# RishWijewardhena/vision-textile-inspection

Measured on AMD Instinct MI355X. Metric: frames/sec whole-node, YOLOv8n-seg 640x640 bs=64; mask IoU vs CPU ref, higher is better.
Workload: dtype f16x2

## Files before the change

vision-textile-inspection_amd/csrc/conv.hip:

```cpp
#include <algorithm>
#include <cstdlib>
#include <type_traits>

#include "conv_dev.h"

namespace vti {

__host__ __device__ inline int patch_dim(int t, int ks, int s, int mode) { return mode == 1 ? t : (t - 1) * s + ks; }

size_t stem_lds_bytes(int TH, int TW);

bool conv_wreg_ok(int ks, int stride, int mode, int WN, int NREP, int threads) {
    return mode == 0 && ks == 1 && stride == 1 && threads == 256 && WN == 4 && NREP <= 4;
}

size_t conv_lds_bytes(int ks, int stride, int mode, int TH, int TW, int WN, int NREP, int wreg) {
    if (mode == 1) return stem_lds_bytes(TH, TW);
    const int npix = patch_dim(TH, ks, stride, mode) * patch_dim(TW, ks, stride, mode);
    const size_t plane = (size_t)((npix + 15) & ~15) * 16;
    const int taps = mode == 1 ? 1 : ks * ks;
    size_t raw = 0;
    if (mode == 1) raw = (((size_t)(2 * TH + 1) * (2 * TW + 1) * 3) + 15) & ~(size_t)15;
    return 4 * plane + (wreg ? 0 : (size_t)WN * NREP * taps * 1024) + raw;
}

template <typename T, int KS, int S, int NREP, int WN, int NREP2 = 0, int NT = 256, bool WREG = false>
__global__ __launch_bounds__(NT, NT == 512 ? 1 : 2) void conv_kernel(const ConvParams p) {
    using vec = typename Tr<T>::vec;
    constexpr int VEC = Tr<T>::VEC, KC = Tr<T>::KC;
    constexpr int TAPS = KS * KS, PAD = KS / 2;
    constexpr int NTB = WN * NREP;
    constexpr int PP = NT / 4;
    constexpr int AR = NT == 512 ? 6 : (S == 2 ? 12 : 8);
    constexpr int BR = (NTB * TAPS * 64 + NT - 1) / NT;
    static_assert(!WREG || (KS == 1 && WN == NT / 64 && NREP2 == 0 && BR == NREP && NREP < 5), "WREG: one consumer wave per fragment");
    constexpr unsigned OOB = 0xFFFFFFFFu;
    extern __shared__ __attribute__((aligned(16))) char smem[];

    const int tid = threadIdx.x, lane = tid & 63, wave = tid >> 6;
    const int wn = wave % WN, wm = wave / WN;
    int t = blockIdx.x;
    const int tx = t % p.tiles_x; t /= p.tiles_x;
    const int ty = t % p.tiles_y;
// ... 127 lines not shown
        if (c < 2) VTI_STAMP(5 + 5 * c);
        if (c + 1 < p.nchunks) __syncthreads();
    };

    issue(0, ra[0], rb[0]);
    if constexpr (PD == 2) {
        if (p.nchunks > 1) issue(1, ra[1], rb[1]);
        for (int c = 0; c < p.nchunks; c += 2) {
            chunk(c, std::integral_constant<int, 0>{});
            if (c + 1 < p.nchunks) chunk(c + 1, std::integral_constant<int, 1>{});
        }
    } else {
        for (int c = 0; c < p.nchunks; ++c) chunk(c, std::integral_constant<int, 0>{});
    }

    VTI_STAMP(11);
    if constexpr (NREP2 == 0) {
        conv_epilogue<T, NREP>(p, acc, pvalid, opy, opx, b, nt0, wn, lane);
    } else {
        static_assert(WN == 1, "fused stage needs the whole Cout in one wave");
        conv_stage2<T, NREP, NREP2>(p, acc, pvalid, opy, opx, b, lane);
    }
    VTI_STAMP(12);
}

size_t convfold_lds_bytes(int TH, int TW) {
    const int npix = (TH + 2) * (TW + 2);
    return 4 * (size_t)((npix + 15) & ~15) * 16 + (size_t)16 * 4 * 1024;
}
bool convfold_supported(int c_in, int c_mid, int c_out, int ntiles2) {
    return c_in == c_mid && c_mid % 16 == 0 && c_out == 64 && c_in % 16 == 0 && c_in <= 64 && combo_has(FoldN2{}, ntiles2);
}

template <typename T, int NREP2, int NT = 256>
__global__ __launch_bounds__(NT, NT == 512 ? 1 : 2) void convfold_kernel(const ConvParams p) {
    using vec = typename Tr<T>::vec;
    constexpr int VEC = Tr<T>::VEC, KC = Tr<T>::KC;
    constexpr int NREP = 4, TAPS = 4, NTB = 16, AR = 8;
    constexpr int BR = NTB * TAPS * 64 / NT;
    constexpr int PPP = NT / 4;
    constexpr unsigned OOB = 0xFFFFFFFFu;
    extern __shared__ __attribute__((aligned(16))) char smem[];

    const int tid = threadIdx.x, lane = tid & 63, wave = (tid >> 6) & 3, mgrp = tid >> 8;
    const int py = wave >> 1, px = wave & 1;
    int t = blockIdx.x;
    const int tx = t % p.tiles_x; t /= p.tiles_x;
    const int ty = t % p.tiles_y;
    const int b = t / p.tiles_y;
    const int oy0 = ty * p.TH, ox0 = tx * p.TW;
    const int PH = p.TH + 2, PW = p.TW + 2;
    const int npix = PH * PW;
    const int plane_bytes = ((npix + 15) & ~15) * 16;
    char* smA = smem;
    char* smB = smem + 4 * plane_bytes;
    const int tile_px = p.TH * p.TW;

    int abase[MREP], opy[MREP], opx[MREP];
    bool pvalid[MREP];
#pragma unroll
    for (int m = 0; m < MREP; ++m) {
        const int pp = (mgrp * MREP + m) * 16 + (lane & 15);
        const bool v = pp < tile_px;
        const int pc = v ? pp : 0;
        const int ly = (int)__umulhi((unsigned)pc, p.tw_magic), lx = pc - ly * p.TW;
        pvalid[m] = v && oy0 + ly < p.Hout && ox0 + lx < p.Wout;
        opy[m] = 2 * (oy0 + ly) + py; opx[m] = 2 * (ox0 + lx) + px;
        abase[m] = (lane >> 4) * plane_bytes + ((ly + py) * PW + lx + px) * 16;
    }
    f32x4 acc[MREP][NREP];
#pragma unroll
    for (int m = 0; m < MREP; ++m)
#pragma unroll
        for (int n = 0; n < NREP; ++n) acc[m][n] = (f32x4){0.f, 0.f, 0.f, 0.f};

    const size_t frame_elems = (size_t)p.Hin * p.Win * p.in_ld;
    const __amdgpu_buffer_rsrc_t rsA = __builtin_amdgcn_make_buffer_rsrc(
        (void*)((const T*)p.in + (size_t)b * frame_elems), 0, (int)(frame_elems * sizeof(T)), 0x00020000);
    const __amdgpu_buffer_rsrc_t rsB = __builtin_amdgcn_make_buffer_rsrc((void*)p.wpk, 0, (int)p.wpk_bytes, 0x00020000);
    const int iy0 = oy0 - 1, ix0 = ox0 - 1;
    const int q = (tid >> 3) & 3;
    const int pix0 = (tid >> 5) * 8 + (tid & 7);
    const int ldsA0 = q * plane_bytes + pix0 * 16;
    const int cvalid = (p.Cin - q * VEC + KC - 1) / KC;
    unsigned aoff[AR];
#pragma unroll
    for (int u = 0; u < AR; ++u) {
        const int pix = pix0 + PPP * u;
        const int ry = (int)__umulhi((unsigned)pix, p.pw_magic), rx = pix - ry * PW;
        const int y = iy0 + ry, x = ix0 + rx;
        const bool ok = pix < npix && (unsigned)y < (unsigned)p.Hin && (unsigned)x < (unsigned)p.Win;
        aoff[u] = ok ? (unsigned)(((y * p.Win + x) * p.in_ld + p.in_coff + q * VEC) * (int)sizeof(T)) : OOB;
    }
    vec ra[AR];
    auto issue = [&](int c) {
        const bool qok = c < cvalid;
#pragma unroll
        for (int u = 0; u < AR; ++u)
            if (pix0 + PPP * u < ((npix + 7) & ~7))
                ra[u] = buf_load16<vec>(rsA, qok ? aoff[u] : OOB, (unsigned)(c * KC * (int)sizeof(T)));
    };
    auto commit = [&](int c) {
        const unsigned sB = (unsigned)((size_t)c * (NTB * TAPS * 1024));
#pragma unroll
        for (int h = 0; h < 2; ++h) {
            vec rb[BR / 2];
#pragma unroll
            for (int u = 0; u < BR / 2; ++u) rb[u] = buf_load16<vec>(rsB, (unsigned)(tid + (h * (BR / 2) + u) * NT) * 16u, sB);
            if (h == 0) {
#pragma unroll
                for (int u = 0; u < AR; ++u)
                    if (pix0 + PPP * u < npix) *(vec*)(smA + ldsA0 + u * (PPP * 16)) = ra[u];
            }
#pragma unroll
            for (int u = 0; u < BR / 2; ++u) *(vec*)(smB + (tid + (h * (BR / 2) + u) * NT) * 16) = rb[u];
        }
    };

    issue(0);
    for (int c = 0; c < p.nchunks; ++c) {
        commit(c);
        __syncthreads();
        if (c + 1 < p.nchunks) issue(c + 1);
        {
            constexpr int NSTEP = TAPS * MREP;
            vec xq[3];
            vec wq[2][NREP];
            auto ldx = [&](int s_) -> vec {
                const int tp = s_ / MREP, mm = s_ % MREP;
                return *(const vec*)(smA + abase[mm] + ((tp >> 1) * PW + (tp & 1)) * 16);
            };
            auto ldw = [&](int tp, vec (&w)[NREP]) {
#pragma unroll
                for (int n = 0; n < NREP; ++n) w[n] = *(const vec*)(smB + ((wave * NREP + n) * TAPS + tp) * 1024 + lane * 16);
            };
            if constexpr (Tr<T>::H2) {
                auto ldw1 = [&](int tp, int n) -> vec { return *(const vec*)(smB + ((wave * NREP + n) * TAPS + tp) * 1024 + lane * 16); };
                h2_taps<NREP, MREP, TAPS, 3>(acc, ldx, ldw1);
            } else {
            ldw(0, wq[0]);
            xq[0] = ldx(0);
            xq[1] = ldx(1);
#pragma unroll
            for (int s_ = 0; s_ < NSTEP; ++s_) {
                const int tp = s_ / MREP, mm = s_ % MREP;
                if (s_ + 2 < NSTEP) xq[(s_ + 2) % 3] = ldx(s_ + 2);
                if (mm == 0 && tp + 1 < TAPS) ldw(tp + 1, wq[(tp + 1) % 2]);
                __builtin_amdgcn_sched_barrier(0);
#pragma unroll
                for (int n = 0; n < NREP; ++n) acc[mm][n] = mma(wq[tp % 2][n], xq[s_ % 3], acc[mm][n]);
                __builtin_amdgcn_sched_barrier(0);
            }
            }
        }
        if (c + 1 < p.nchunks) __syncthreads();
    }
    conv_stage2<T, NREP, NREP2, true>(p, acc, pvalid, opy, opx, b, lane);
}

hipError_t launch_convfold(int dtype, const ConvParams& p, size_t lds_bytes, hipStream_t st) {
    dim3 grid((unsigned)(p.B * p.tiles_y * p.tiles_x));
    if (grid.x == 0) return hipSuccess;
    const int nthr = p.nt == 512 ? 512 : 256;
    if (p.TH * p.TW > (nthr / 256) * MREP * 16 || ((p.TH + 2) * (p.TW + 2) + 7) / 8 * 32 > nthr * 8 || p.Cout != 256 || !p.out2 || !p.fold)
        return hipErrorInvalidValue;
    return with_conv_type(dtype, [&](auto t) -> hipError_t {
        using T = typename decltype(t)::type;
        if (p.nt == 512) {
            if constexpr (sizeof(T) == 4)
                return combo_dispatch(FoldN2{}, [&](auto c) {
                    return launch_lds<convfold_kernel<T, decltype(c)::v[0], 512>>(grid, dim3(512), lds_bytes, st, p);
                }, p.ntiles2);
            return hipErrorInvalidValue;
        }
        return combo_dispatch(FoldN2{}, [&](auto c) {
            return launch_lds<convfold_kernel<T, decltype(c)::v[0]>>(grid, dim3(256), lds_bytes, st, p);
        }, p.ntiles2);
    });
}

template <typename T, int NREP>
__global__ __launch_bounds__(256) void stem_kernel(const ConvParams p) {
    using vec = typename Tr<T>::vec;
    constexpr int VEC = Tr<T>::VEC, KC = Tr<T>::KC;
    constexpr int NCH = 32 / KC;
    extern __shared__ __attribute__((aligned(16))) char smem[];
    T* lut = (T*)smem;
    unsigned* raw32 = (unsigned*)(smem + 1024);
    const unsigned char* raw = (const unsigned char*)raw32;

    const int tid = threadIdx.x, lane = tid & 63, wave = tid >> 6;
    int t = blockIdx.x;
    const int tx = t % p.tiles_x; t /= p.tiles_x;
    const int ty = t % p.tiles_y;
    const int b = t / p.tiles_y;
    const int oy0 = ty * p.TH, ox0 = tx * p.TW;
    const int RH = 2 * p.TH + 1, RWB = (2 * p.TW + 1) * 3;
    const int RWD = (RWB + 6) >> 2;
    const int pitch = RWD * 4;
    const int x0b = (ox0 * 2 - 1) * 3, a0 = x0b & ~3, shift = x0b - a0;
    const int y0 = oy0 * 2 - 1;
    const uint8_t* inb = (const uint8_t*)p.in + (size_t)b * p.Hin * p.Win * 3;
    const int rowbytes = p.Win * 3;
    if ((rowbytes & 3) == 0 && RH * RWD <= 8 * 256) {
// ... 50 lines not shown
    f32x4 acc[MREP][NREP];
#pragma unroll
    for (int m = 0; m < MREP; ++m)
#pragma unroll
        for (int n = 0; n < NREP; ++n) acc[m][n] = (f32x4){0.f, 0.f, 0.f, 0.f};
#pragma unroll
    for (int c = 0; c < NCH; ++c) {
        int off[VEC];
#pragma unroll
        for (int j = 0; j < VEC; ++j) {
            const int k = c * KC + (lane >> 4) * VEC + j;
            const int tap = k / 3, chn = k - tap * 3;
            const int kh = tap / 3, kw = tap - kh * 3;
            off[j] = k < 27 ? kh * pitch + kw * 3 + (p.swap_rb ? 2 - chn : chn) : -1;
        }
        vec w[NREP];
#pragma unroll
        for (int n = 0; n < NREP; ++n) {
            const int nt = nt0 + n < p.ntiles_n ? nt0 + n : 0;
            w[n] = ((const vec*)p.wpk)[((size_t)c * p.ntiles_n + nt) * 64 + lane];
        }
#pragma unroll
        for (int m = 0; m < MREP; ++m) {
            vec x;
#pragma unroll
            for (int j = 0; j < VEC; ++j) vset<T>(x, j, off[j] >= 0 ? lut[raw[rbase[m] + off[j]]] : to_T<T>(0.f));
#pragma unroll
            for (int n = 0; n < NREP; ++n) acc[m][n] = mma(w[n], x, acc[m][n]);
        }
    }
    conv_epilogue<T, NREP>(p, acc, pvalid, opy, opx, b, nt0, 0, lane);
}

constexpr int SL_TH = 8, SL_TW = 40;
constexpr int SL_SH = 2 * SL_TH + 1, SL_SW = 2 * SL_TW + 1, SL_NSP = SL_SH * SL_SW;
constexpr int SL_RH = 4 * SL_TH + 3, SL_RWB = (4 * SL_TW + 3) * 3, SL_RWD = (SL_RWB + 6) >> 2;
constexpr int sl_pitch(int es) { return es == 2 ? 520 : 512; }
constexpr int SL_NJ = (SL_SW + 3) / 4, SL_NWIN = SL_SH * SL_NJ;
static_assert(24 * (SL_NJ - 1) + 32 <= 512 && SL_RWD * 4 <= 512, "stem windows must stay inside a patch row");

size_t stem_l1_lds_bytes(int dtype) {
    const size_t es = dtype == VTI_F16 ? 2 : 4, pes = dtype == VTI_F32 ? 4 : 2;
    return (((size_t)SL_RH * sl_pitch((int)pes) * pes + 15) & ~(size_t)15) + (size_t)SL_NSP * 16 * es;
}

template <typename T>
__global__ __launch_bounds__(256, sizeof(T) == 2 ? 2 : 1) void stem_l1_kernel(const ConvParams p) {
    using vec = typename Tr<T>::vec;
    constexpr int ES = (int)sizeof(T);
    constexpr bool XH = Tr<T>::H2;
    using PT = typename std::conditional<XH, half_t, T>::type;
    using pvec = typename Tr<PT>::vec;
    constexpr int VEC = Tr<PT>::VEC, KC = Tr<PT>::KC, PES = (int)sizeof(PT);
    constexpr int NCH = 32 / KC;
    constexpr int NWP = XH ? 2 : 1;
    constexpr int NS1 = sizeof(T) == 2 ? 5 : 9;
    constexpr bool FAST = !Tr<T>::F32;
    constexpr int SL_PITCH = sl_pitch(PES);
    constexpr int CP_BYTES = (SL_RH * SL_PITCH * PES + 15) & ~15;
    extern __shared__ __attribute__((aligned(16))) char smem[];
    PT* cp = (PT*)smem;
    char* sout = smem + CP_BYTES;

    const int tid = threadIdx.x, lane = tid & 63, wave = tid >> 6, g = lane >> 4;
    const int ntiles = p.B * p.tiles_y * p.tiles_x;
    if ((int)blockIdx.x >= ntiles) return;
    const int Hs = (p.Hin - 1) / 2 + 1, Ws = (p.Win - 1) / 2 + 1;
    const int rowbytes = p.Win * 3;
    auto tile_geom = [&](int tt, int& b_, int& oy0_, int& ox0_) {
        const int tx = tt % p.tiles_x, r = tt / p.tiles_x;
        b_ = r / p.tiles_y; oy0_ = (r % p.tiles_y) * SL_TH; ox0_ = tx * SL_TW;
    };
    VTI_STAMP(0);
    constexpr int RC = (SL_RWD + 63) / 64, NR = (SL_RH + 3) / 4;
    unsigned vv[NR][RC];
    const bool aligned = (rowbytes & 3) == 0;
    auto issue_raw = [&](int tt) {
        int b_, oy0_, ox0_;
        tile_geom(tt, b_, oy0_, ox0_);
        const int iy0_ = 2 * (2 * oy0_ - 1) - 1, a0_ = ((2 * (2 * ox0_ - 1) - 1) * 3) & ~3;
        const uint8_t* inb_ = (const uint8_t*)p.in + (size_t)b_ * p.Hin * p.Win * 3;
#pragma unroll
        for (int it = 0; it < NR; ++it) {
            const int ry = wave + 4 * it;
            const int y = iy0_ + ry;
            const bool row_ok = ry < SL_RH && (unsigned)y < (unsigned)p.Hin;
#pragma unroll
            for (int ch = 0; ch < RC; ++ch) {
                const int rd = lane + 64 * ch;
                const int gx = a0_ + 4 * rd;
                const bool ok = row_ok && rd < SL_RWD && gx >= 0 && gx < rowbytes;
                vv[it][ch] = *(const unsigned*)(inb_ + (ok ? (size_t)y * rowbytes + gx : (size_t)0));
            }
        }
    };
    if (aligned) issue_raw((int)blockIdx.x);
    for (int t = (int)blockIdx.x; t < ntiles; t += (int)gridDim.x) {
    int b, oy0, ox0;
    tile_geom(t, b, oy0, ox0);
    const int sy0 = 2 * oy0 - 1, sx0 = 2 * ox0 - 1;
    const int iy0 = 2 * sy0 - 1;
    const int x0b = (2 * sx0 - 1) * 3, a0 = x0b & ~3;
    const uint8_t* inb = (const uint8_t*)p.in + (size_t)b * p.Hin * p.Win * 3;
    const void* w0p = p.w0;
    const void* w1p = p.wpk;
    asm volatile("" : "+s"(w0p), "+s"(w1p));
    pvec wA[4][3][NCH * NWP];
    {
        const pvec* w0 = (const pvec*)w0p + (size_t)(p.swap_rb ? 1 : 0) * (4 * 3 * NCH * NWP * 64);
#pragma unroll
        for (int pp = 0; pp < 4; ++pp)
#pragma unroll
            for (int kh = 0; kh < 3; ++kh)
#pragma unroll
                for (int c = 0; c < NCH * NWP; ++c) wA[pp][kh][c] = w0[(size_t)((pp * 3 + kh) * NCH * NWP + c) * 64 + lane];
    }
    vec w1all[NS1][2];
#pragma unroll
    for (int s1 = 0; s1 < NS1; ++s1)
#pragma unroll
        for (int n = 0; n < 2; ++n) w1all[s1][n] = ((const vec*)w1p)[((size_t)s1 * 2 + n) * 64 + lane];
    const f32x4 bias0_4 = *(const f32x4*)(p.bias0 + g * 4);
    Stage2Regs<T, 2, 2> s2r;
    if (p.out2) stage2_preload<T, 2, 2>(p, lane, false, s2r);
    {
        if (aligned) {
#pragma unroll
            for (int it = 0; it < NR; ++it) {
                const int ry = wave + 4 * it;
// ... 23 lines not shown
                        for (int k = 0; k < 4; ++k)
                            if (gx + k >= 0 && gx + k < rowbytes) v |= (unsigned)inb[(size_t)y * rowbytes + gx + k] << (8 * k);
                    }
                    vv[it][ch] = v;
                }
            }
        }
#pragma unroll
        for (int it = 0; it < NR; ++it) {
            const int ry = wave + 4 * it;
#pragma unroll
            for (int ch = 0; ch < RC; ++ch) {
                const int rd = lane + 64 * ch;
                if (ry >= SL_RH || rd >= SL_RWD) continue;
                const unsigned v = vv[it][ch];
                PT* o = cp + (size_t)ry * SL_PITCH + 4 * rd;
                if constexpr (XH) {
                    half4 hv;
#pragma unroll
                    for (int k = 0; k < 4; ++k) hv[k] = (half_t)(float)((v >> (8 * k)) & 0xffu);
                    *(half4*)o = hv;
                } else if constexpr (sizeof(T) == 2) {
                    half4 hv;
#pragma unroll
                    for (int k = 0; k < 4; ++k) hv[k] = (half_t)((float)((v >> (8 * k)) & 0xffu) * (1.0f / 255.0f));
                    *(half4*)o = hv;
                } else {
#pragma unroll
                    for (int k = 0; k < 4; ++k) o[k] = to_T<T>((float)((v >> (8 * k)) & 0xffu) / 255.0f);
                }
            }
        }
    }
    for (int i = tid; i < SL_RH * ((SL_PITCH - 4 * SL_RWD) / 4); i += 256) {
        const int ry = i / ((SL_PITCH - 4 * SL_RWD) / 4), c4 = i - ry * ((SL_PITCH - 4 * SL_RWD) / 4);
        PT* o = cp + (size_t)ry * SL_PITCH + 4 * SL_RWD + 4 * c4;
        o[0] = to_T<PT>(0.f); o[1] = to_T<PT>(0.f); o[2] = to_T<PT>(0.f); o[3] = to_T<PT>(0.f);
    }
    __syncthreads();
    VTI_STAMP(1);
    if (aligned && t + (int)gridDim.x < ntiles) issue_raw(t + (int)gridDim.x);
    {
        const f32x4 bias4 = bias0_4;
        constexpr int NBLK = (SL_NWIN + 15) / 16;
        for (int blk = wave; blk < NBLK; blk += 4) {
            const int wi = blk * 16 + (lane & 15);
            const bool wvalid = wi < SL_NWIN;
            const int wc = wvalid ? wi : SL_NWIN - 1;
            const int J = wc / SL_SH, sy = wc - J * SL_SH;
            const PT* base = cp + (size_t)(2 * sy) * SL_PITCH + 24 * J + g * VEC;
            pvec x[3][NCH];
#pragma unroll
            for (int kh = 0; kh < 3; ++kh)
#pragma unroll
                for (int c = 0; c < NCH; ++c) x[kh][c] = *(const pvec*)(base + kh * SL_PITCH + c * KC);
            f32x4 acc[4];
#pragma unroll
            for (int pp = 0; pp < 4; ++pp) {
                acc[pp] = (f32x4){0.f, 0.f, 0.f, 0.f};
#pragma unroll
                for (int kh = 0; kh < 3; ++kh)
#pragma unroll
                    for (int c = 0; c < NCH; ++c)
#pragma unroll
                        for (int wp = 0; wp < NWP; ++wp) acc[pp] = mma(wA[pp][kh][c * NWP + wp], x[kh][c], acc[pp]);
            }
            const bool row_in = (unsigned)(sy0 + sy) < (unsigned)Hs;
#pragma unroll
            for (int pp = 0; pp < 4; ++pp) {
                const int sx = 4 * J + pp;
                f32x4 v = silu4<FAST>(acc_bias<T>(acc[pp], bias4, p.alpha0));
                if (!(row_in && (unsigned)(sx0 + sx) < (unsigned)Ws)) v = (f32x4){0.f, 0.f, 0.f, 0.f};
                if (wvalid && sx < SL_SW) {
                    T* o = (T*)(sout + ((size_t)(sy * SL_SW + sx) * 16 + g * 4) * ES);
                    if constexpr (sizeof(T) == 2) {
                        half4 hv;
#pragma unroll
                        for (int j = 0; j < 4; ++j) hv[j] = (half_t)v[j];
                        *(half4*)o = hv;
                    } else {
                        *(u32x4*)o = pack4<T>(v);
                    }
                }
            }
        }
    }
    __syncthreads();
    VTI_STAMP(2);
    int opy[MREP], opx[MREP], sbase[MREP];
    bool pvalid[MREP];
#pragma unroll
    for (int m = 0; m < MREP; ++m) {
        const int pp = (wave * MREP + m) * 16 + (lane & 15);
        const int py = pp / SL_TW, px = pp - py * SL_TW;
        opy[m] = oy0 + py; opx[m] = ox0 + px;
        pvalid[m] = opy[m] < p.Hout && opx[m] < p.Wout;
        sbase[m] = ((2 * py) * SL_SW + 2 * px) * 16 * ES;
    }
    f32x4 acc[MREP][2];
#pragma unroll
    for (int m = 0; m < MREP; ++m) { acc[m][0] = (f32x4){0.f, 0.f, 0.f, 0.f}; acc[m][1] = (f32x4){0.f, 0.f, 0.f, 0.f}; }
#pragma unroll
    for (int s = 0; s < NS1; ++s) {
        const int tap = sizeof(T) == 2 ? 2 * s + (g >> 1) : s;
        const int tc = tap < 9 ? tap : 8;
        const int toff = ((tc / 3) * SL_SW + (tc % 3)) * 16 * ES + (sizeof(T) == 2 ? (g & 1) * 8 : g * 4) * ES;
        vec w1[2];
#pragma unroll
        for (int n = 0; n < 2; ++n) w1[n] = w1all[s][n];
#pragma unroll
        for (int m = 0; m < MREP; ++m) {
            const vec x = *(const vec*)(sout + sbase[m] + toff);
#pragma unroll
            for (int n = 0; n < 2; ++n) acc[m][n] = mma(w1[n], x, acc[m][n]);
        }
    }
    VTI_STAMP(3);
    if (p.out2) conv_stage2<T, 2, 2, false, true>(p, acc, pvalid, opy, opx, b, lane, &s2r);
    else conv_epilogue<T, 2>(p, acc, pvalid, opy, opx, b, 0, 0, lane);
    VTI_STAMP(12);
    }
}

void stem_l1_tile(int* th, int* tw) { *th = SL_TH; *tw = SL_TW; }

int stem_l1_grid(int dtype, int ntiles, bool persistent) {
    const int wgpc = (int)std::min<size_t>(2, (160 * 1024) / stem_l1_lds_bytes(dtype));
    if (!persistent) return ntiles;
    return std::min(ntiles, 256 * std::max(1, wgpc));
}

hipError_t launch_stem_l1(int dtype, const ConvParams& p, hipStream_t st, bool persistent) {
    dim3 grid((unsigned)stem_l1_grid(dtype, p.B * p.tiles_y * p.tiles_x, persistent));
    if (grid.x == 0) return hipSuccess;
    const size_t lds = stem_l1_lds_bytes(dtype);
    return with_conv_type(dtype, [&](auto t) { return launch_lds<stem_l1_kernel<typename decltype(t)::type>>(grid, dim3(256), lds, st, p); });
}

size_t stem_lds_bytes(int TH, int TW) { return 1024 + (size_t)(2 * TH + 1) * ((((2 * TW + 1) * 3 + 6) >> 2) * 4); }

using ConvTile3 = Combos<Ints<1, 1>, Ints<2, 1>, Ints<3, 1>, Ints<4, 1>, Ints<5, 1>, Ints<1, 2>, Ints<2, 2>, Ints<1, 4>>;
using ConvTile1 = decltype(concat(ConvTile3{}, Combos<Ints<3, 2>, Ints<4, 2>, Ints<5, 2>, Ints<2, 4>, Ints<3, 4>, Ints<4, 4>, Ints<5, 4>>{}));
using ConvTile1W = Combos<Ints<1, 4>, Ints<2, 4>, Ints<3, 4>, Ints<4, 4>>;
using StemNrep = Combos<Ints<1>, Ints<2>, Ints<3>, Ints<4>, Ints<5>>;

// ... 66 lines not shown
```

vision-textile-inspection_amd/csrc/conv_dev.h:

```cpp
#pragma once
#include "vti_internal.h"

namespace vti {

typedef _Float16 half_t;
typedef _Float16 half8 __attribute__((ext_vector_type(8)));
typedef _Float16 half4 __attribute__((ext_vector_type(4)));
typedef float f32x4 __attribute__((ext_vector_type(4)));

typedef unsigned u32x4 __attribute__((ext_vector_type(4)));

struct h2_t { unsigned u; };
struct h2x4 { u32x4 u; };
constexpr float H2_SX = 16.0f;

template <typename T> struct Tr;
template <> struct Tr<half_t> { typedef half8 vec; static constexpr int VEC = 8, KC = 32; static constexpr bool H16 = true, F32 = false, H2 = false; };
template <> struct Tr<float> { typedef f32x4 vec; static constexpr int VEC = 4, KC = 16; static constexpr bool H16 = false, F32 = true, H2 = false; };
template <> struct Tr<h2_t> { typedef h2x4 vec; static constexpr int VEC = 4, KC = 16; static constexpr bool H16 = false, F32 = false, H2 = true; };

typedef _Float16 half2v __attribute__((ext_vector_type(2)));
__device__ __forceinline__ unsigned h2_enc(float v) {
    half2v p;
    p[0] = (half_t)__builtin_fmaf(v, H2_SX, 0.0f);
// ... 316 lines not shown
                } else {
                    v += unpack4<T>(*(const u32x4*)rp);
                }
            }
            const size_t o = opix * p.out_ld + p.out_coff + co;
            if (p.scalar_store) {
#pragma unroll
                for (int j = 0; j < 4; ++j) {
                    if (cout0 + j < p.Cout) {
                        if (p.out_f32) ((float*)p.out)[o + j] = v[j];
                        else if constexpr (Tr<T>::H2) ((unsigned*)p.out)[o + j] = h2_enc(v[j]);
                        else ((T*)p.out)[o + j] = (T)v[j];
                    }
                }
            } else if (p.out_f32 || Tr<T>::F32) {
                *(f32x4*)((float*)p.out + o) = v;
            } else if constexpr (Tr<T>::H2) {
                *(u32x4*)((unsigned*)p.out + o) = pack4<T>(v);
            } else {
                half4 hv;
#pragma unroll
                for (int j = 0; j < 4; ++j) hv[j] = (half_t)v[j];
                *(half4*)((half_t*)p.out + o) = hv;
            }
        }
    }
}

template <typename V> __device__ __forceinline__ V buf_load16(__amdgpu_buffer_rsrc_t r, unsigned voff, unsigned soff) {
    const u32x4 v = __builtin_amdgcn_raw_buffer_load_b128(r, voff, soff, 0);
    return __builtin_bit_cast(V, v);
}

template <typename T, int NREP, int NREP2> struct Stage2Regs {
    using vec = typename Tr<T>::vec;
    static constexpr int KT = sizeof(T) == 2 ? (NREP + 1) / 2 : NREP;
    vec w2[KT][NREP2];
    f32x4 bias1[NREP];
    f32x4 bias2[NREP2];
};

template <typename T, int NREP, int NREP2>
__device__ __forceinline__ void stage2_preload(const ConvParams& p, int lane, bool fold, Stage2Regs<T, NREP, NREP2>& r) {
    using vec = typename Tr<T>::vec;
    const __amdgpu_buffer_rsrc_t rsW2 = __builtin_amdgcn_make_buffer_rsrc(
        (void*)p.w2, 0, (int)(Stage2Regs<T, NREP, NREP2>::KT * p.ntiles2 * 1024), 0x00020000);
#pragma unroll
    for (int t2 = 0; t2 < Stage2Regs<T, NREP, NREP2>::KT; ++t2)
#pragma unroll
        for (int n = 0; n < NREP2; ++n) r.w2[t2][n] = buf_load16<vec>(rsW2, (unsigned)(((t2 * p.ntiles2 + n) * 64 + lane) * 16), 0u);
    const float* b1 = p.bias + (fold ? 4 * (16 * NREP) : 0) + (lane >> 4) * 4 * NREP;
#pragma unroll
    for (int n = 0; n < NREP; ++n) r.bias1[n] = *(const f32x4*)(b1 + 4 * n);
    const int crun2 = p.nat2 ? (lane >> 4) * 4 : (lane >> 4) * 4 * NREP2, cstep2 = p.nat2 ? 16 : 4;
#pragma unroll
    for (int n = 0; n < NREP2; ++n) r.bias2[n] = *(const f32x4*)(p.bias2 + crun2 + cstep2 * n);
}

template <typename T, int NREP, int NREP2, bool FOLD = false, bool PRE = false>
__device__ __forceinline__ void conv_stage2(const ConvParams& p, f32x4 (&acc)[MREP][NREP], const bool (&pvalid)[MREP],
                                            const int (&opy)[MREP], const int (&opx)[MREP], int b, int lane,
                                            const Stage2Regs<T, NREP, NREP2>* pre = nullptr, bool interior = false) {
    const int OW = FOLD ? 2 * p.Wout : p.Wout;
    using vec = typename Tr<T>::vec;
    constexpr bool FAST = !Tr<T>::F32;
    constexpr int KT = sizeof(T) == 2 ? (NREP + 1) / 2 : NREP;
// ... 215 lines not shown
```

vision-textile-inspection_amd/csrc/conv_pk.hip:

```cpp
#include <algorithm>
#include <cstdlib>
#include <type_traits>

#include "conv_dev.h"

namespace vti {

constexpr int PK_PWP = 24;
constexpr int PK_TW = 20;
constexpr int PK_ROWS = 4;
constexpr int PK_MAXD = 9;
constexpr int PK_MAXD2 = 13;

using ConvPkS1 = Combos<Ints<1, 1>, Ints<2, 1>, Ints<3, 1>, Ints<4, 1>, Ints<5, 1>, Ints<1, 2>, Ints<2, 2>, Ints<3, 2>, Ints<4, 2>, Ints<1, 4>,
                        Ints<2, 4>>;
using ConvPkS2 = Combos<Ints<1, 4>, Ints<2, 2>, Ints<4, 1>, Ints<2, 1>, Ints<1, 2>>;
using Conv1Pk = decltype(concat(ConvPkS1{}, Combos<Ints<4, 4>>{}));
bool conv_pk_instantiated(int nrep, int wn) { return combo_has(ConvPkS1{}, nrep, wn); }
bool conv_pk2_instantiated(int nrep, int wn) { return combo_has(ConvPkS2{}, nrep, wn); }
bool conv1_pk_instantiated(int nrep, int wn) { return combo_has(Conv1Pk{}, nrep, wn); }
using Conv1PkWH2 = Combos<Ints<2, 2, 4>, Ints<2, 2, 6>, Ints<2, 2, 8>, Ints<2, 2, 12>, Ints<2, 2, 16>,
                          Ints<2, 4, 4>, Ints<2, 4, 6>, Ints<2, 4, 8>, Ints<2, 4, 12>, Ints<2, 4, 16>>;
using Conv1PkWF16 = Combos<Ints<2, 2, 2>, Ints<2, 2, 3>, Ints<2, 2, 4>, Ints<2, 2, 6>, Ints<2, 2, 8>,
                           Ints<2, 4, 2>, Ints<2, 4, 3>, Ints<2, 4, 4>, Ints<2, 4, 6>, Ints<2, 4, 8>, Ints<4, 1, 2>>;
// ... 5 lines not shown

static size_t pk_stage_bytes(int TH, int S) { return S == 2 ? (size_t)(2 * TH + 1) * 2 * PK_PWP * 64 : (size_t)(TH + 2) * PK_PWP * 64; }
static size_t pk3_lds_bytes(int S, int TH, int WN, int NREP, int nchunks, int depth, int wstat) {
    const int nwbuf = wstat ? nchunks : nchunks > 2 ? depth : (nchunks > 1 ? 2 : 1);
    return depth * pk_stage_bytes(TH, S) + (size_t)nwbuf * WN * NREP * 9 * 1024 + (size_t)WN * NREP * 16 * 4;
}
static bool pk3_fits(int S, int TH, int WN, int NREP, int nchunks, int wstat) {
    if (TH % PK_ROWS || (S == 2 && !conv_pk2_instantiated(NREP, WN))) return false;
    const int ncomp = (TH / PK_ROWS) * WN;
    if (ncomp < 1 || ncomp > 4) return false;
    const int ndma = (int)(pk_stage_bytes(TH, S) / 1024);
    if ((ndma + ncomp - 1) / ncomp > (S == 2 ? PK_MAXD2 : PK_MAXD)) return false;
    return pk3_lds_bytes(S, TH, WN, NREP, nchunks, 2, wstat) <= 160 * 1024;
}
template <typename F>
static int pk_ring_depth(int maxd, int per_step, F lds_at) {
    int d = 2;
    while (d < maxd && lds_at(d + 1) <= 160 * 1024 && per_step * (d - 1) <= 63) ++d;
    return d;
}
static int pk3_depth(int S, int TH, int WN, int NREP, int nchunks, int wstat, int maxd) {
    if (!pk3_fits(S, TH, WN, NREP, nchunks, wstat)) return 0;
    const int ncomp = (TH / PK_ROWS) * WN;
    const int per_step = ((int)(pk_stage_bytes(TH, S) / 1024) + ncomp - 1) / ncomp + (nchunks > 2 && !wstat ? (WN * NREP * 9 + ncomp - 1) / ncomp : 0);
    return pk_ring_depth(maxd, per_step, [&](int d) { return pk3_lds_bytes(S, TH, WN, NREP, nchunks, d, wstat); });
}
size_t conv_pk_lds_bytes(int TH, int WN, int NREP, int nchunks, int depth, int wstat) { return pk3_lds_bytes(1, TH, WN, NREP, nchunks, depth, wstat); }
size_t conv_pk2_lds_bytes(int TH, int WN, int NREP, int nchunks, int depth, int wstat) { return pk3_lds_bytes(2, TH, WN, NREP, nchunks, depth, wstat); }
bool conv_pk_fits(int TH, int WN, int NREP, int nchunks, int wstat) { return pk3_fits(1, TH, WN, NREP, nchunks, wstat); }
bool conv_pk2_fits(int TH, int WN, int NREP, int nchunks, int wstat) { return pk3_fits(2, TH, WN, NREP, nchunks, wstat); }
int conv_pk_depth(int TH, int WN, int NREP, int nchunks, int wstat, int maxd) { return pk3_depth(1, TH, WN, NREP, nchunks, wstat, maxd); }
int conv_pk2_depth(int TH, int WN, int NREP, int nchunks, int wstat, int maxd) { return pk3_depth(2, TH, WN, NREP, nchunks, wstat, maxd); }

__device__ __forceinline__ void dma16(__amdgpu_buffer_rsrc_t r, unsigned voff, unsigned soff, unsigned lds_addr) {
    unsigned keep;
    asm volatile("s_mov_b32 %0, m0\n\ts_mov_b32 m0, %1\n\ts_nop 0\n\tbuffer_load_dwordx4 %2, %3, %4 offen lds\n\ts_mov_b32 m0, %0"
                 : "=&s"(keep) : "s"(lds_addr), "v"(voff), "s"(r), "s"(soff) : "memory");
}

template <int N> __device__ __forceinline__ void wait_vm() { asm volatile("s_waitcnt vmcnt(%0)" :: "i"(N) : "memory"); }
template <int N> struct WaitVm { static __device__ __forceinline__ void go(int n) { if (n >= N) wait_vm<N>(); else WaitVm<N - 1>::go(n); } };
template <> struct WaitVm<0> { static __device__ __forceinline__ void go(int) { wait_vm<0>(); } };

__device__ __forceinline__ void pk_stagger_wait(int units) {
    if (units > 0 && (int)(blockIdx.x >> 3) * 2 >= (int)(gridDim.x >> 3))
        for (int i = 0; i < units; ++i) __builtin_amdgcn_s_sleep(16);
}

template <typename T, int NREP, int WN, int NREP2 = 0, bool FOLD = false, int S = 1>
__global__ __launch_bounds__(512) void conv3_pk(const ConvParams p) {
    using vec = typename Tr<T>::vec;
    constexpr int VEC = Tr<T>::VEC, KC = Tr<T>::KC, ES = (int)sizeof(T);
    constexpr int TAPS = FOLD ? 4 : 9, NTB = WN * NREP;
    constexpr int PWP = S == 2 ? 2 * PK_PWP : PK_PWP;
    constexpr int MAXD = S == 2 ? PK_MAXD2 : PK_MAXD;
    static_assert(S == 1 || (S == 2 && !FOLD && NREP2 == 0), "stride 2: plain epilogue only");
    constexpr int WCHUNK = NTB * TAPS * 1024;
    constexpr unsigned OOB = 0x80000000u;
    constexpr bool FAST = !Tr<T>::F32;
    extern __shared__ __attribute__((aligned(16))) char smem[];

    const int tid = threadIdx.x, lane = tid & 63;
    const int wave = __builtin_amdgcn_readfirstlane(tid >> 6);
    static_assert(!FOLD || (WN == 4 && NREP2 > 0), "fold: one compute wave per output phase, fused 1x1 epilogue");
    const int ncomp = (p.TH / PK_ROWS) * WN;
    const int nld = (int)(blockDim.x >> 6) - ncomp;
    const int PH = S == 2 ? 2 * p.TH + 1 : p.TH + 2;
    const int stage_bytes = PH * PWP * 64;
    const int ndma = PH * PWP / 16;
    const int D = p.pk_depth;
    const bool stream_w = p.nchunks > 2 && !p.pk_wstat;
    const int wbuf_off = D * stage_bytes;
    const int bias_off = wbuf_off + (stream_w ? D : p.nchunks) * WCHUNK;
// ... 1195 lines not shown
```

vision-textile-inspection_amd/csrc/vti_api.cpp:

```cpp
#include <algorithm>
#include <cmath>
#include <cstdio>
#include <cstdlib>
#include <cstring>
#include <new>

#include "vti_internal.h"
#include "rawframes_dev.h"

using namespace vti;

struct vti_ctx {
    Options opt;
    Plan plan;
    std::string err;
    int device = -1;
    void* d_wpk = nullptr;
    float* d_bias = nullptr;
    std::vector<float> alpha;
    char* ws = nullptr;
    size_t ws_bytes = 0;
    size_t act_bytes = 0;
    const void* last_input = nullptr;
    void* last_proto = nullptr;
// ... 500 lines not shown
                }
                stem_l1_tile(&q.TH, &q.TW);
                q.tiles_y = (q.Hout + q.TH - 1) / q.TH; q.tiles_x = (q.Wout + q.TW - 1) / q.TW; q.WN = 1;
                q.scalar_store = scalar_store(q.Cout, q.out_ld, q.out_coff);
#ifdef VTI_STAMPS
                if (r.name == run.stamp_op)
                    stamped_launch(q, (size_t)stem_l1_grid(dt, B * q.tiles_y * q.tiles_x, !run.stem_not_persistent), false, st,
                                   ("[stamps] op " + r.name + " + layer 1 (1: patch staged, 2: stem done, 3: layer-1 MFMAs done, 12: end)").c_str(),
                                   [&] { return launch_stem_l1(dt, q, st, !run.stem_not_persistent); });
#endif
                VTI_HIP(c, launch_stem_l1(dt, q, st, !run.stem_not_persistent), "stem + layer 1");
                break;
            }
            if (op.fold >= 0) {
                const ConvRow& ru = P.convs[op.fold];
                ConvParams q;
                memset(&q, 0, sizeof q);
                q.in = buf_ptr(c, op.in.buf, input, proto); q.B = B; q.Hin = ru.h_in; q.Win = ru.w_in; q.Hout = ru.h_in; q.Wout = ru.w_in;
                q.Cin = ru.c1; q.in_ld = ib.C; q.in_coff = op.in.coff; q.Cout = g.gemm_n; q.act = 1; q.fold = 1; q.pk_lin = run.pk_linear_map;
                q.TH = g.TH; q.TW = g.TW; q.tiles_y = (q.Hout + g.TH - 1) / g.TH; q.tiles_x = (q.Wout + g.TW - 1) / g.TW; q.WN = 4; q.nt = g.threads;
                q.nchunks = g.nchunks; q.ntiles_n = g.ntiles_n;
                q.pw_magic = (unsigned)((0x100000000ull + (unsigned)(g.TW + 2) - 1) / (unsigned)(g.TW + 2));
                q.tw_magic = (unsigned)((0x100000000ull + (unsigned)g.TW - 1) / (unsigned)g.TW);
                q.wpk = (const char*)c->d_wpk + g.wpk_off; q.bias = c->d_bias + g.bias_off; q.wpk_bytes = (unsigned)packed_fold_bytes(g);
                q.alpha = c->alpha[op.conv]; q.alpha0 = 1.f;
                fill_stage2(c, q, op, input, proto);
                if (g.pk) {
                    q.pk = 1; q.pk_depth = g.pk_depth; q.in_bytes = (unsigned)((size_t)B * q.Hin * q.Win * q.in_ld * P.esize);
                    q.pk_tiles = B * q.tiles_y * q.tiles_x;
                    q.pk_wgs = pk_grid(q.pk_tiles, 1, 1, run.pk_max_wgs);
                    q.pk_xcd = q.pk_wgs >= 8 ? 1 : 0;
                    VTI_HIP(c, launch_conv_pk_fold(dt, q, g.lds, st), r.name.c_str());
                } else {
                    VTI_HIP(c, launch_convfold(dt, q, g.lds, st), r.name.c_str());
                }
                break;
            }
            ConvParams p;
            fill_conv_params(run, P.esize, p, r, g, B, buf_ptr(c, op.in.buf, input, proto), ib.C, op.in.coff,
                             buf_ptr(c, op.out.buf, input, proto), ob.C, op.out.coff,
                             op.has_res ? buf_ptr(c, op.res.buf, input, proto) : nullptr,
                             op.has_res ? P.bufs[op.res.buf].C : 0, op.res.coff,
                             (const char*)c->d_wpk + g.wpk_off, c->d_bias + g.bias_off, op.out_f32, swap_rb);
            p.alpha = c->alpha[op.conv]; p.alpha0 = 1.f;
            p.pk_stagger *= stagger_units(run, dt);
            p.alpha2 = op.pair >= 0 ? c->alpha[op.pair] : 1.f;
            if (op.fused >= 0) {
                fill_stage2(c, p, op, input, proto);
                if (op.pred_mode) {
                    const int no = 4 + P.desc.nc + P.desc.nm;
                    p.out2 = pred + (size_t)op.pred_a0 * no;
                    p.out2_ld = no; p.out2_coff = op.pred_cbase; p.out2_f32 = 1; p.out2_bstride = P.num_anchors;
                    p.act2 = op.pred_mode == 2 ? 2 : op.pred_mode == 3 ? 3 : 0;
                    p.dfl_stride = (float)op.dfl_stride;
                    p.scalar_store2 = scalar_store(g.gemm_n2, no, op.pred_cbase);
                    p.best = (op.pred_mode == 2 && best) ? best + (size_t)op.pred_a0 * 2 : nullptr;
                }
            }
            if (op.pair >= 0) {
                p.w2 = (const char*)c->d_wpk + g.wpk_off2;
                p.bias2 = c->d_bias + g.bias_off2;
                if (p.pk != 3) return fail(c, VTI_ERR_UNSUPPORTED, "fused bottleneck needs the persistent kernel (tensor too large?)");
                if (op.tail >= 0) {
                    const Buf& o2 = P.bufs[op.out2.buf];
                    if (dt == VTI_F16) p.in_coff -= r.c1;
                    p.alpha0 = c->alpha[op.tail];
// ... 1598 lines not shown
```

Measured before the change: 16650.

## Double-buffer folded conv operands in LDS with async buffer-to-LDS weight DMA

Adds a double-buffered variant of the 512-thread folded conv kernel. Two LDS images hold activation planes and weights. The next chunk's weights are fetched with direct buffer_load...lds DMA interleaved into the MMA loop, and activations are committed after compute, which removes one barrier per chunk. The goal is to hide global load latency behind the matrix math. The cost is twice the LDS footprint, which may lower occupancy, plus reliance on inline asm that manipulates M0. Timing stamps are also added for probing.

```diff
diff --git a/vision-textile-inspection_amd/csrc/conv.hip b/vision-textile-inspection_amd/csrc/conv.hip
--- a/vision-textile-inspection_amd/csrc/conv.hip
+++ b/vision-textile-inspection_amd/csrc/conv.hip
@@ -9,6 +9,13 @@
 __host__ __device__ inline int patch_dim(int t, int ks, int s, int mode) { return mode == 1 ? t : (t - 1) * s + ks; }
 
 size_t stem_lds_bytes(int TH, int TW);
+
+constexpr size_t kLdsPerCu = 160 * 1024;
+#ifdef VTI_CONV_SINGLE_IMAGE
+constexpr bool kConvSecondImage = false;
+#else
+constexpr bool kConvSecondImage = true;
+#endif
 
 bool conv_wreg_ok(int ks, int stride, int mode, int WN, int NREP, int threads) {
     return mode == 0 && ks == 1 && stride == 1 && threads == 256 && WN == 4 && NREP <= 4;
@@ -202,7 +209,7 @@
     return c_in == c_mid && c_mid % 16 == 0 && c_out == 64 && c_in % 16 == 0 && c_in <= 64 && combo_has(FoldN2{}, ntiles2);
 }
 
-template <typename T, int NREP2, int NT = 256>
+template <typename T, int NREP2, int NT = 256, bool DB = false>
 __global__ __launch_bounds__(NT, NT == 512 ? 1 : 2) void convfold_kernel(const ConvParams p) {
     using vec = typename Tr<T>::vec;
     constexpr int VEC = Tr<T>::VEC, KC = Tr<T>::KC;
@@ -222,9 +229,11 @@
     const int PH = p.TH + 2, PW = p.TW + 2;
     const int npix = PH * PW;
     const int plane_bytes = ((npix + 15) & ~15) * 16;
-    char* smA = smem;
-    char* smB = smem + 4 * plane_bytes;
+    static_assert(!DB || NT == 512, "second operand image: the 512-thread kernel");
+    constexpr int WIMG = NTB * TAPS * 1024;
+    const int image_bytes = 4 * plane_bytes + WIMG;
     const int tile_px = p.TH * p.TW;
+    VTI_STAMP(0);
 
     int abase[MREP], opy[MREP], opx[MREP];
     bool pvalid[MREP];
@@ -270,34 +279,60 @@
             if (pix0 + PPP * u < ((npix + 7) & ~7))
                 ra[u] = buf_load16<vec>(rsA, qok ? aoff[u] : OOB, (unsigned)(c * KC * (int)sizeof(T)));
     };
-    auto commit = [&](int c) {
-        const unsigned sB = (unsigned)((size_t)c * (NTB * TAPS * 1024));
+    auto commit_a = [&](char* smA) {
+#pragma unroll
+        for (int u = 0; u < AR; ++u)
+            if (pix0 + PPP * u < npix) *(vec*)(smA + ldsA0 + u * (PPP * 16)) = ra[u];
+    };
+    auto commit = [&](int c, char* smA, char* smB) {
+        const unsigned sB = (unsigned)((size_t)c * WIMG);
 #pragma unroll
         for (int h = 0; h < 2; ++h) {
             vec rb[BR / 2];
 #pragma unroll
             for (int u = 0; u < BR / 2; ++u) rb[u] = buf_load16<vec>(rsB, (unsigned)(tid + (h * (BR / 2) + u) * NT) * 16u, sB);
-            if (h == 0) {
-#pragma unroll
-                for (int u = 0; u < AR; ++u)
-                    if (pix0 + PPP * u < npix) *(vec*)(smA + ldsA0 + u * (PPP * 16)) = ra[u];
-            }
+            if (h == 0) commit_a(smA);
 #pragma unroll
             for (int u = 0; u < BR / 2; ++u) *(vec*)(smB + (tid + (h * (BR / 2) + u) * NT) * 16) = rb[u];
         }
     };
 
     issue(0);
+    if constexpr (DB) {
+        const unsigned dst = (unsigned)(size_t)(__attribute__((address_space(3))) char*)smem + (unsigned)(4 * plane_bytes);
+        for (int f = __builtin_amdgcn_readfirstlane(tid >> 6); f < NTB * TAPS; f += NT / 64)
+            dma16(rsB, (unsigned)lane * 16u, (unsigned)(f * 1024), dst + (unsigned)(f * 1024));
+        commit_a(smem);
+        wait_vm_all();
+        __syncthreads();
+    }
     for (int c = 0; c < p.nchunks; ++c) {
-        commit(c);
-        __syncthreads();
+        char* const smA = smem + (DB ? (c & 1) * image_bytes : 0);
+        char* const smB = smA + 4 * plane_bytes;
+        if (c < 2) VTI_STAMP(1 + 5 * c);
+        if constexpr (!DB) {
+            commit(c, smA, smB);
+            if (c < 2) VTI_STAMP(3 + 5 * c);
+            __syncthreads();
+        }
+        if (c < 2) VTI_STAMP(4 + 5 * c);
         if (c + 1 < p.nchunks) issue(c + 1);
+        constexpr int NDMA = NTB * TAPS / (NT / 64);
+        static_assert(!DB || (NTB * TAPS % (NT / 64) == 0 && NDMA + 2 <= TAPS * MREP), "one weight fragment per wave and step");
+        const int wave8 = __builtin_amdgcn_readfirstlane(tid >> 6);
+        const unsigned dma_voff = c + 1 < p.nchunks ? (unsigned)lane * 16u : OOB;
+        const unsigned dma_src = (unsigned)((c + 1) * WIMG + wave8 * 1024);
+        const unsigned dma_dst = (unsigned)(size_t)(__attribute__((address_space(3))) char*)smem +
+                                 (unsigned)(((c + 1) & 1) * image_bytes + 4 * plane_bytes + wave8 * 1024);
         {
             constexpr int NSTEP = TAPS * MREP;
             vec xq[3];
             vec wq[2][NREP];
             auto ldx = [&](int s_) -> vec {
                 const int tp = s_ / MREP, mm = s_ % MREP;
+                if constexpr (DB) {
+                    if (s_ >= 2 && s_ < 2 + NDMA) dma16(rsB, dma_voff, dma_src + (unsigned)((s_ - 2) * (NT / 64) * 1024), dma_dst + (unsigned)((s_ - 2) * (NT / 64) * 1024));
+                }
                 return *(const vec*)(smA + abase[mm] + ((tp >> 1) * PW + (tp & 1)) * 16);
             };
             auto ldw = [&](int tp, vec (&w)[NREP]) {
@@ -323,9 +358,16 @@
             }
             }
         }
+        if (c < 2) VTI_STAMP(5 + 5 * c);
+        if constexpr (DB) {
+            if (c + 1 < p.nchunks) commit_a(smem + ((c + 1) & 1) * image_bytes);
+            wait_vm_all();
+        }
         if (c + 1 < p.nchunks) __syncthreads();
     }
+    VTI_STAMP(11);
     conv_stage2<T, NREP, NREP2, true>(p, acc, pvalid, opy, opx, b, lane);
+    VTI_STAMP(12);
 }
 
 hipError_t launch_convfold(int dtype, const ConvParams& p, size_t lds_bytes, hipStream_t st) {
@@ -334,12 +376,15 @@
     const int nthr = p.nt == 512 ? 512 : 256;
     if (p.TH * p.TW > (nthr / 256) * MREP * 16 || ((p.TH + 2) * (p.TW + 2) + 7) / 8 * 32 > nthr * 8 || p.Cout != 256 || !p.out2 || !p.fold)
         return hipErrorInvalidValue;
+    const size_t image = convfold_lds_bytes(p.TH, p.TW);
+    const bool db = p.nt == 512 && kConvSecondImage && 2 * image <= kLdsPerCu;
     return with_conv_type(dtype, [&](auto t) -> hipError_t {
         using T = typename decltype(t)::type;
         if (p.nt == 512) {
             if constexpr (sizeof(T) == 4)
                 return combo_dispatch(FoldN2{}, [&](auto c) {
-                    return launch_lds<convfold_kernel<T, decltype(c)::v[0], 512>>(grid, dim3(512), lds_bytes, st, p);
+                    return db ? launch_lds<convfold_kernel<T, decltype(c)::v[0], 512, true>>(grid, dim3(512), std::max(lds_bytes, 2 * image), st, p)
+                              : launch_lds<convfold_kernel<T, decltype(c)::v[0], 512>>(grid, dim3(512), lds_bytes, st, p);
                 }, p.ntiles2);
             return hipErrorInvalidValue;
         }
diff --git a/vision-textile-inspection_amd/csrc/conv_dev.h b/vision-textile-inspection_amd/csrc/conv_dev.h
--- a/vision-textile-inspection_amd/csrc/conv_dev.h
+++ b/vision-textile-inspection_amd/csrc/conv_dev.h
@@ -372,6 +372,18 @@
     return __builtin_bit_cast(V, v);
 }
 
+__device__ __forceinline__ void dma16(__amdgpu_buffer_rsrc_t r, unsigned voff, unsigned soff, unsigned lds_addr) {
+    unsigned keep;
+    asm volatile("s_mov_b32 %0, m0\n\ts_mov_b32 m0, %1\n\ts_nop 0\n\tbuffer_load_dwordx4 %2, %3, %4 offen lds\n\ts_mov_b32 m0, %0"
+                 : "=&s"(keep) : "s"(lds_addr), "v"(voff), "s"(r), "s"(soff) : "memory");
+}
+
+template <int N> __device__ __forceinline__ void wait_vm() { asm volatile("s_waitcnt vmcnt(%0)" :: "i"(N) : "memory"); }
+__device__ __forceinline__ void wait_vm_all() {
+    __builtin_amdgcn_s_waitcnt(0x0F70);
+    asm volatile("" ::: "memory");
+}
+
 template <typename T, int NREP, int NREP2> struct Stage2Regs {
     using vec = typename Tr<T>::vec;
     static constexpr int KT = sizeof(T) == 2 ? (NREP + 1) / 2 : NREP;
diff --git a/vision-textile-inspection_amd/csrc/conv_pk.hip b/vision-textile-inspection_amd/csrc/conv_pk.hip
--- a/vision-textile-inspection_amd/csrc/conv_pk.hip
+++ b/vision-textile-inspection_amd/csrc/conv_pk.hip
@@ -61,13 +61,6 @@
 int conv_pk_depth(int TH, int WN, int NREP, int nchunks, int wstat, int maxd) { return pk3_depth(1, TH, WN, NREP, nchunks, wstat, maxd); }
 int conv_pk2_depth(int TH, int WN, int NREP, int nchunks, int wstat, int maxd) { return pk3_depth(2, TH, WN, NREP, nchunks, wstat, maxd); }
 
-__device__ __forceinline__ void dma16(__amdgpu_buffer_rsrc_t r, unsigned voff, unsigned soff, unsigned lds_addr) {
-    unsigned keep;
-    asm volatile("s_mov_b32 %0, m0\n\ts_mov_b32 m0, %1\n\ts_nop 0\n\tbuffer_load_dwordx4 %2, %3, %4 offen lds\n\ts_mov_b32 m0, %0"
-                 : "=&s"(keep) : "s"(lds_addr), "v"(voff), "s"(r), "s"(soff) : "memory");
-}
-
-template <int N> __device__ __forceinline__ void wait_vm() { asm volatile("s_waitcnt vmcnt(%0)" :: "i"(N) : "memory"); }
 template <int N> struct WaitVm { static __device__ __forceinline__ void go(int n) { if (n >= N) wait_vm<N>(); else WaitVm<N - 1>::go(n); } };
 template <> struct WaitVm<0> { static __device__ __forceinline__ void go(int) { wait_vm<0>(); } };
 
diff --git a/vision-textile-inspection_amd/csrc/vti_api.cpp b/vision-textile-inspection_amd/csrc/vti_api.cpp
--- a/vision-textile-inspection_amd/csrc/vti_api.cpp
+++ b/vision-textile-inspection_amd/csrc/vti_api.cpp
@@ -556,6 +556,12 @@
                     q.pk_xcd = q.pk_wgs >= 8 ? 1 : 0;
                     VTI_HIP(c, launch_conv_pk_fold(dt, q, g.lds, st), r.name.c_str());
                 } else {
+#ifdef VTI_STAMPS
+                    if (r.name == run.stamp_op &&
+                        stamped_launch(q, (size_t)B * q.tiles_y * q.tiles_x, false, st, ("[stamps] op " + r.name + " (per-tile fold)").c_str(),
+                                       [&] { return launch_convfold(dt, q, g.lds, st); }))
+                        break;
+#endif
                     VTI_HIP(c, launch_convfold(dt, q, g.lds, st), r.name.c_str());
                 }
                 break;
```

Result: slower. 16490 (-1.0%).

## Split stem output LDS into even/odd column planes with XOR swizzle

Applied to the files above, without the earlier changes.

For the half-pair input path, the stem's LDS output buffer is reorganised so even and odd columns sit in separate planes, and 16-byte pieces are XOR-swizzled. The stride-2 layer-1 reads then hit consecutive slots, which should cut LDS bank conflicts. The one-time zeroing of the patch-row padding is hoisted out of the persistent tile loop, since that region is never overwritten. The extra address arithmetic for swizzling and plane indexing is the cost, and the layout must stay consistent between the producer and consumer stages.

```diff
diff --git a/vision-textile-inspection_amd/csrc/conv.hip b/vision-textile-inspection_amd/csrc/conv.hip
--- a/vision-textile-inspection_amd/csrc/conv.hip
+++ b/vision-textile-inspection_amd/csrc/conv.hip
@@ -3,6 +3,7 @@
 #include <type_traits>
 
 #include "conv_dev.h"
+#include "stem_tile.h"
 
 namespace vti {
 
@@ -456,11 +457,9 @@
     conv_epilogue<T, NREP>(p, acc, pvalid, opy, opx, b, nt0, 0, lane);
 }
 
-constexpr int SL_TH = 8, SL_TW = 40;
-constexpr int SL_SH = 2 * SL_TH + 1, SL_SW = 2 * SL_TW + 1, SL_NSP = SL_SH * SL_SW;
+static_assert(SL_MREP == MREP, "stem_tile.h's m-tiles per wave are conv_dev.h's");
 constexpr int SL_RH = 4 * SL_TH + 3, SL_RWB = (4 * SL_TW + 3) * 3, SL_RWD = (SL_RWB + 6) >> 2;
 constexpr int sl_pitch(int es) { return es == 2 ? 520 : 512; }
-constexpr int SL_NJ = (SL_SW + 3) / 4, SL_NWIN = SL_SH * SL_NJ;
 static_assert(24 * (SL_NJ - 1) + 32 <= 512 && SL_RWD * 4 <= 512, "stem windows must stay inside a patch row");
 
 size_t stem_l1_lds_bytes(int dtype) {
@@ -485,6 +484,7 @@
     extern __shared__ __attribute__((aligned(16))) char smem[];
     PT* cp = (PT*)smem;
     char* sout = smem + CP_BYTES;
+    constexpr bool PL = XH;
 
     const int tid = threadIdx.x, lane = tid & 63, wave = tid >> 6, g = lane >> 4;
     const int ntiles = p.B * p.tiles_y * p.tiles_x;
@@ -519,6 +519,11 @@
         }
     };
     if (aligned) issue_raw((int)blockIdx.x);
+    for (int i = tid; i < SL_RH * ((SL_PITCH - 4 * SL_RWD) / 4); i += 256) {
+        const int ry = i / ((SL_PITCH - 4 * SL_RWD) / 4), c4 = i - ry * ((SL_PITCH - 4 * SL_RWD) / 4);
+        PT* o = cp + (size_t)ry * SL_PITCH + 4 * SL_RWD + 4 * c4;
+        o[0] = to_T<PT>(0.f); o[1] = to_T<PT>(0.f); o[2] = to_T<PT>(0.f); o[3] = to_T<PT>(0.f);
+    }
     for (int t = (int)blockIdx.x; t < ntiles; t += (int)gridDim.x) {
     int b, oy0, ox0;
     tile_geom(t, b, oy0, ox0);
@@ -608,11 +613,6 @@
             }
         }
     }
-    for (int i = tid; i < SL_RH * ((SL_PITCH - 4 * SL_RWD) / 4); i += 256) {
-        const int ry = i / ((SL_PITCH - 4 * SL_RWD) / 4), c4 = i - ry * ((SL_PITCH - 4 * SL_RWD) / 4);
-        PT* o = cp + (size_t)ry * SL_PITCH + 4 * SL_RWD + 4 * c4;
-        o[0] = to_T<PT>(0.f); o[1] = to_T<PT>(0.f); o[2] = to_T<PT>(0.f); o[3] = to_T<PT>(0.f);
-    }
     __syncthreads();
     VTI_STAMP(1);
     if (aligned && t + (int)gridDim.x < ntiles) issue_raw(t + (int)gridDim.x);
@@ -623,7 +623,7 @@
             const int wi = blk * 16 + (lane & 15);
             const bool wvalid = wi < SL_NWIN;
             const int wc = wvalid ? wi : SL_NWIN - 1;
-            const int J = wc / SL_SH, sy = wc - J * SL_SH;
+            const int J = stem_tile::win_col(wc), sy = stem_tile::win_row(wc);
             const PT* base = cp + (size_t)(2 * sy) * SL_PITCH + 24 * J + g * VEC;
             pvec x[3][NCH];
 #pragma unroll
@@ -642,13 +642,16 @@
                         for (int wp = 0; wp < NWP; ++wp) acc[pp] = mma(wA[pp][kh][c * NWP + wp], x[kh][c], acc[pp]);
             }
             const bool row_in = (unsigned)(sy0 + sy) < (unsigned)Hs;
+            const int so0 = stem_tile::slot(PL, sy, 4 * J);
+            const int obase = PL ? stem_tile::piece_lin(so0, g) : (so0 * 16 + g * 4) * ES;
 #pragma unroll
             for (int pp = 0; pp < 4; ++pp) {
                 const int sx = 4 * J + pp;
                 f32x4 v = silu4<FAST>(acc_bias<T>(acc[pp], bias4, p.alpha0));
                 if (!(row_in && (unsigned)(sx0 + sx) < (unsigned)Ws)) v = (f32x4){0.f, 0.f, 0.f, 0.f};
                 if (wvalid && sx < SL_SW) {
-                    T* o = (T*)(sout + ((size_t)(sy * SL_SW + sx) * 16 + g * 4) * ES);
+                    T* o = (T*)(sout + (PL ? stem_tile::piece_swz_at(obase, stem_tile::win_slot(true, pp))
+                                           : obase + stem_tile::win_slot(false, pp) * 16 * ES));
                     if constexpr (sizeof(T) == 2) {
                         half4 hv;
 #pragma unroll
@@ -671,7 +674,7 @@
         const int py = pp / SL_TW, px = pp - py * SL_TW;
         opy[m] = oy0 + py; opx[m] = ox0 + px;
         pvalid[m] = opy[m] < p.Hout && opx[m] < p.Wout;
-        sbase[m] = ((2 * py) * SL_SW + 2 * px) * 16 * ES;
+        sbase[m] = PL ? stem_tile::piece_lin(stem_tile::l1_slot(true, py, px), g) : stem_tile::l1_slot(false, py, px) * 16 * ES;
     }
     f32x4 acc[MREP][2];
 #pragma unroll
@@ -680,13 +683,14 @@
     for (int s = 0; s < NS1; ++s) {
         const int tap = sizeof(T) == 2 ? 2 * s + (g >> 1) : s;
         const int tc = tap < 9 ? tap : 8;
-        const int toff = ((tc / 3) * SL_SW + (tc % 3)) * 16 * ES + (sizeof(T) == 2 ? (g & 1) * 8 : g * 4) * ES;
+        const int toff = PL ? stem_tile::tap_slot(true, tc / 3, tc % 3)
+                            : stem_tile::tap_slot(false, tc / 3, tc % 3) * 16 * ES + (sizeof(T) == 2 ? (g & 1) * 8 : g * 4) * ES;
         vec w1[2];
 #pragma unroll
         for (int n = 0; n < 2; ++n) w1[n] = w1all[s][n];
 #pragma unroll
         for (int m = 0; m < MREP; ++m) {
-            const vec x = *(const vec*)(sout + sbase[m] + toff);
+            const vec x = *(const vec*)(sout + (PL ? stem_tile::piece_swz_at(sbase[m], toff) : sbase[m] + toff));
 #pragma unroll
             for (int n = 0; n < 2; ++n) acc[m][n] = mma(w1[n], x, acc[m][n]);
         }
diff --git a/vision-textile-inspection_amd/csrc/stem_tile.h b/vision-textile-inspection_amd/csrc/stem_tile.h
--- /dev/null
+++ b/vision-textile-inspection_amd/csrc/stem_tile.h
@@ -0,0 +1,37 @@
+#pragma once
+
+#ifndef VTI_HD
+#define VTI_HD __host__ __device__
+#endif
+
+namespace vti {
+
+constexpr int SL_TH = 8, SL_TW = 40;
+constexpr int SL_SH = 2 * SL_TH + 1, SL_SW = 2 * SL_TW + 1, SL_NSP = SL_SH * SL_SW;
+constexpr int SL_NJ = (SL_SW + 3) / 4, SL_NWIN = SL_SH * SL_NJ;
+constexpr int SL_EVEN = (SL_SW + 1) / 2;
+constexpr int SL_MREP = SL_TH * SL_TW / 64;
+static_assert(SL_SW % 8 == 1, "8 consecutive stem rows must be 8 consecutive slots mod 8");
+static_assert(SL_TH * SL_TW % 64 == 0, "layer 1's tile must split into whole m-tiles over 4 waves");
+
+namespace stem_tile {
+
+VTI_HD constexpr int win_col(int wi) { return wi / SL_SH; }
+VTI_HD constexpr int win_row(int wi) { return wi % SL_SH; }
+
+VTI_HD constexpr int l1_pixel(int wave, int m, int i) { return (wave * SL_MREP + m) * 16 + i; }
+
+VTI_HD constexpr int slot(bool planes, int sy, int sx) {
+    return planes ? sy * SL_SW + (sx & 1) * SL_EVEN + (sx >> 1) : sy * SL_SW + sx;
+}
+VTI_HD constexpr int tap_slot(bool planes, int kh, int kw) { return slot(planes, kh, kw); }
+VTI_HD constexpr int win_slot(bool planes, int pp) { return slot(planes, 0, pp); }
+VTI_HD constexpr int l1_slot(bool planes, int py, int px) { return slot(planes, 2 * py, 2 * px); }
+
+VTI_HD constexpr int piece_lin(int s, int g) { return 64 * s + 16 * g; }
+VTI_HD constexpr int piece_swz(int lin) { return lin ^ ((lin >> 3) & 0x30); }
+VTI_HD constexpr int piece_swz_at(int lin, int d) { return (lin ^ (((lin + 64 * d) >> 3) & 0x30)) + 64 * d; }
+VTI_HD constexpr int piece_off(bool planes, int s, int g) { return planes ? piece_swz(piece_lin(s, g)) : piece_lin(s, g); }
+
+}
+}
```

After: 15730 before, 15800 after, median of 6. About the same (+0.4%).
